# tahaspc82442/federated_multi_modal

Measured on AMD Instinct MI355X. Metric: images/sec/node (ViT-B/16 MaPLe fwd+bwd), higher is better.
Workload: dtype fp16; 1 GPU; c4: PatternNet-shape 38-class synthetic, J=9, batch=32 per client (configs[3]); clients=1, batch_per_client=32, global_batch=32, classes=38, prompt_depth=9, n_ctx=2, parallelism=one federated client per GPU x1, FedAvg all-reduce per round, round=512 local steps + 1 FedAvg, hipgraph=True

## Files before the change

federated_multi_modal_amd/_lib.py:

```python
from __future__ import annotations

import ctypes
import os
from pathlib import Path

_HERE = Path(__file__).resolve().parent
LIB_PATH = _HERE / "lib" / "libmapfed.so"

P, I, L, F = ctypes.c_void_p, ctypes.c_int, ctypes.c_int64, ctypes.c_float

SIGNATURES = {
    "mf_abi_version": [],
    "mf_gemm_nt": [P, L, P, L, P, L, I, I, I, P, P, P, L, I, I, P],
    "mf_gemm": [P, L, I, P, L, I, P, L, I, I, I, P, P, P, L, I, I, P],
    "mf_layernorm_fwd": [P, L, P, P, P, P, L, P, P, I, I, P],
    "mf_layernorm_bwd_blocks": [I],
    "mf_layernorm_bwd": [P, L, P, L, P, P, P, P, P, L, P, L, P, P, P, I, I, I, P],
    "mf_col_reduce_desc_bytes": [],
    "mf_col_reduce_batch": [P, I, I, P],
    "mf_attention_fwd": [P, L, P, L, P, I, I, I, I, I, P],
    "mf_attention_fwd_rows": [P, L, P, L, P, I, I, I, I, I, I, P],
    "mf_attention_bwd": [P, L, P, L, P, L, P, P, I, P, L, I, I, I, I, P],
    "mf_qkv_attention_fwd": [P, L, I, P, P, P, L, P, L, P, I, I, I, I, I, P],
    "mf_qkv_attention_supported": [I, I, I, I],
    "mf_im2col_patch": [P, I, P, I, I, I, P],
    "mf_vision_assemble": [P, P, P, P, P, I, I, I, I, P],
    "mf_text_assemble": [P, P, P, P, P, I, I, I, I, P],
    "mf_prompt_inject_fwd": [P, P, I, I, I, I, I, P],
    "mf_prompt_inject_bwd": [P, I, I, I, I, I, P, I, I, I, P],
    "mf_transpose_f16": [P, L, P, L, I, I, P],
    "mf_colsum_blocks": [I],
    "mf_colsum_f16": [P, L, I, I, P, I, P, P],
    "mf_cast_f16_f32": [P, P, L, P],
    "mf_small_linear_fwd": [P, P, P, P, I, I, I, I, P],
    "mf_small_linear_bwd": [P, P, P, P, P, P, I, I, I, I, I, P],
    "mf_gemm_splitk_ws_floats": [I, I, I, I],
    "mf_small_linear_desc_bytes": [],
# ... 37 lines not shown
_LIB = None


class MapfedError(RuntimeError):
    pass


def lib():
    global _LIB
    if _LIB is not None:
        return _LIB
    path = os.environ.get("MAPFED_LIB", str(LIB_PATH))
    if not os.path.exists(path):
        raise MapfedError(f"libmapfed.so not found at {path}: run __graft_entry__.build() "
                          "(make -C federated_multi_modal_amd/csrc)")
    h = ctypes.CDLL(path)
    h.mf_last_error.restype = ctypes.c_char_p
    h.mf_last_error.argtypes = []
    for name, args in SIGNATURES.items():
        fn = getattr(h, name)
        fn.argtypes = args
        fn.restype = _RESTYPES.get(name, ctypes.c_int)
    _LIB = h
    return h


def exported_symbols():
    return ["mf_last_error"] + list(SIGNATURES)


# ... 9 lines not shown
```

federated_multi_modal_amd/csrc/attention.hip:

```cpp
#include <algorithm>
#include <cstdlib>

#include "mf_common.h"

namespace {

MF_DEV int sw_off(int row, int col) {
  return row * 64 + ((((col >> 3) ^ (row & 7))) << 3) + (col & 7);
}

MF_DEV f16x4 tr_read(const f16* img, int r0, int c0, int lane) {
  const int ii = lane & 15;
  const int row = r0 + (ii >> 2);
  const int col = c0 + 4 * (ii & 3);
  const f16* p = img + sw_off(row, col);
  s16x4 v = __builtin_amdgcn_ds_read_tr16_b64_v4i16((__attribute__((address_space(3))) s16x4*)(p));
  return __builtin_bit_cast(f16x4, v);
}

MF_DEV f16x8 cat8(f16x4 a, f16x4 b) {
  return (f16x8){a[0], a[1], a[2], a[3], b[0], b[1], b[2], b[3]};
}

MF_DEV f16x8 ld_frag(const f16* img, int row, int chunk) {
  return *(const f16x8*)(img + row * 64 + ((chunk ^ (row & 7)) << 3));
}

typedef __attribute__((address_space(3))) void* lds_ptr_t;
template <int LP>
MF_DEV void stage_rows(f16* img, const f16* base, int64_t ld, int L, int col0) {
  const int lane = threadIdx.x & 63, w = threadIdx.x >> 6, nw = blockDim.x >> 6;
  const int lrow = lane >> 3, lchunk = (lane & 7) ^ lrow;
  for (int i = w; i < LP / 8; i += nw) {
    int row = i * 8 + lrow;
    row = row < L ? row : L - 1;
    __builtin_amdgcn_global_load_lds((const void*)(base + (int64_t)row * ld + col0 + lchunk * 8),
                                     (lds_ptr_t)(img + i * 8 * 64), 16, 0, 0);
  }
}
MF_DEV void stage_wait() {
  __builtin_amdgcn_s_waitcnt((0 & 15) | (7 << 4) | (15 << 8));
  __syncthreads();
}

constexpr float kScale = 0.125f;

#ifdef MF_ATTN_STAMPS
__device__ unsigned long long* g_astamps;
#define MF_ASTAMP(slot)                                                                   \
  do {                                                                                    \
    if (threadIdx.x == 0 && blockIdx.y == 0) g_astamps[(size_t)blockIdx.x * 8 + (slot)] = __builtin_amdgcn_s_memrealtime(); \
  } while (0)
// ... 609 lines not shown
}

template <int LP>
struct BwdLds {
  static constexpr int P = LP + 8;
  static constexpr int ELEMS = 2 * LP * 64 + LP * P + 2 * LP * 2;
};

MF_DEV f16x4 tr_read_p(const f16* img, int pitch, int r0, int c0, int lane) {
  const int ii = lane & 15;
  const f16* p = img + (r0 + (ii >> 2)) * pitch + c0 + 4 * (ii & 3);
  s16x4 v = __builtin_amdgcn_ds_read_tr16_b64_v4i16((__attribute__((address_space(3))) s16x4*)(p));
  return __builtin_bit_cast(f16x4, v);
}

template <int LP, bool CAUSAL, int KT>
__global__ __launch_bounds__(64 * (LP / (16 * KT))) void attn_bwd_fused_kernel(
    const f16* __restrict__ qkv, int64_t ld_qkv, const f16* __restrict__ out, int64_t ld_out,
    const f16* __restrict__ dout, int64_t ld_dout, const float* __restrict__ lse, int ld_lse,
    f16* __restrict__ dqkv, int64_t ld_dqkv, int L, int H) {
  constexpr int PT = BwdLds<LP>::P;
  __shared__ __attribute__((aligned(16))) f16 smem[BwdLds<LP>::ELEMS];
  f16* sQ = smem;
  f16* sdO = smem + LP * 64;
  f16* sdST = smem + 2 * LP * 64;
  float* sL = (float*)(sdST + LP * PT);
  float* sD = sL + LP;

  const int D = H * 64;
  const int nh = blockIdx.x, n = nh / H, h = nh % H;
  const f16* base = qkv + (int64_t)n * L * ld_qkv;
  const f16* obase = out + (int64_t)n * L * ld_out;
  const f16* dobase = dout + (int64_t)n * L * ld_dout;
  MF_ASTAMP(0);
  stage_rows<LP>(sQ, base, ld_qkv, L, h * 64);
  stage_rows<LP>(sdO, dobase, ld_dout, L, h * 64);

  const int lane = threadIdx.x & 63, w = threadIdx.x >> 6;
  const int fr = lane & 15, fg = lane >> 4;
  {
    constexpr int LPQ = 4 / KT, DPL = 64 / LPQ;
    const int q = 16 * KT * w + lane / LPQ;
    const int part = lane % LPQ;
    float d = 0.f;
    if (q < L) {
      const f16* o = obase + (int64_t)q * ld_out + h * 64 + DPL * part;
      const f16* g = dobase + (int64_t)q * ld_dout + h * 64 + DPL * part;
#pragma unroll
      for (int c = 0; c < DPL / 8; ++c) {
        f16x8 a = *(const f16x8*)(o + 8 * c), b = *(const f16x8*)(g + 8 * c);
#pragma unroll
        for (int e = 0; e < 8; ++e) d += (float)a[e] * (float)b[e];
      }
    }
#pragma unroll
    for (int o2 = 1; o2 < LPQ; o2 <<= 1) d += __shfl_xor(d, o2, 64);
    if (part == 0) {
      sD[q] = q < L ? d : 0.f;
      sL[q] = q < L ? lse[(int64_t)nh * ld_lse + q] * 1.4426950408889634f : INFINITY;
    }
  }
  const int k0 = 16 * KT * w;
  f16x8 kf[KT][2], vf[KT][2];
#pragma unroll
  for (int kt = 0; kt < KT; ++kt) {
    const int key = k0 + 16 * kt + fr;
    const int kc = key < L ? key : L - 1;
#pragma unroll
    for (int s2 = 0; s2 < 2; ++s2) {
      kf[kt][s2] = *(const f16x8*)(base + (int64_t)kc * ld_qkv + D + h * 64 + 32 * s2 + 8 * fg);
      vf[kt][s2] = *(const f16x8*)(base + (int64_t)kc * ld_qkv + 2 * D + h * 64 + 32 * s2 + 8 * fg);
    }
  }
  stage_wait();
  MF_ASTAMP(1);

  f32x4 dv[KT][4], dk[KT][4];
#pragma unroll
  for (int kt = 0; kt < KT; ++kt)
#pragma unroll
    for (int dt = 0; dt < 4; ++dt) dv[kt][dt] = dk[kt][dt] = (f32x4){0.f, 0.f, 0.f, 0.f};
#pragma unroll 1
  for (int qp = 0; qp < LP / 32; ++qp) {
    if (CAUSAL && 32 * qp + 31 < k0) continue;
    f16x8 pf[KT], dsf[KT];
#pragma unroll
    for (int a = 0; a < 2; ++a) {
      const int qt = 2 * qp + a;
      f32x4 sacc[KT], pacc[KT];
#pragma unroll
      for (int kt = 0; kt < KT; ++kt) sacc[kt] = pacc[kt] = (f32x4){0.f, 0.f, 0.f, 0.f};
#pragma unroll
      for (int s2 = 0; s2 < 2; ++s2) {
        const f16x8 qfr = ld_frag(sQ, qt * 16 + fr, 4 * s2 + fg);
        const f16x8 ofr = ld_frag(sdO, qt * 16 + fr, 4 * s2 + fg);
#pragma unroll
        for (int kt = 0; kt < KT; ++kt) {
          sacc[kt] = __builtin_amdgcn_mfma_f32_16x16x32_f16(qfr, kf[kt][s2], sacc[kt], 0, 0, 0);
// ... 57 lines not shown
    const int row = k0 + 16 * kt + fr;
#pragma unroll
    for (int s2 = 0; s2 < 2; ++s2) *(f16x8*)(sQ + row * 64 + (((4 * s2 + fg) ^ (row & 7)) << 3)) = kf[kt][s2];
  }
  __syncthreads();
  MF_ASTAMP(3);
  const f16* sK = sQ;
  const int q0 = 16 * KT * w;
  f32x4 dq[KT][4];
#pragma unroll
  for (int qt = 0; qt < KT; ++qt)
#pragma unroll
    for (int dt = 0; dt < 4; ++dt) dq[qt][dt] = (f32x4){0.f, 0.f, 0.f, 0.f};
#pragma unroll 1
  for (int ks = 0; ks < LP / 32; ++ks) {
    if (CAUSAL && 32 * ks > q0 + 16 * KT - 1) break;
    f16x8 dsf[KT];
#pragma unroll
    for (int qt = 0; qt < KT; ++qt)
      dsf[qt] = cat8(tr_read_p(sdST, PT, 32 * ks + 4 * fg, q0 + 16 * qt, lane),
                     tr_read_p(sdST, PT, 32 * ks + 16 + 4 * fg, q0 + 16 * qt, lane));
#pragma unroll
    for (int dt = 0; dt < 4; ++dt) {
      const f16x8 ak = cat8(tr_read(sK, 32 * ks + 4 * fg, 16 * dt, lane), tr_read(sK, 32 * ks + 16 + 4 * fg, 16 * dt, lane));
#pragma unroll
      for (int qt = 0; qt < KT; ++qt) dq[qt][dt] = __builtin_amdgcn_mfma_f32_16x16x32_f16(ak, dsf[qt], dq[qt][dt], 0, 0, 0);
    }
  }
#pragma unroll
  for (int qt = 0; qt < KT; ++qt) {
// ... 188 lines not shown
  attn_bwd_dkv_kernel<P, false><<<grid, block, 0, st>>>((const f16*)qkv, ld_qkv, (const f16*)dout, ld_dout, lse,     \
                                                      dq_dot_ws, ld_lse, (f16*)dqkv, ld_dqkv, L, H);               \
  attn_bwd_dq_kernel<P, false><<<grid, block, 0, st>>>((const f16*)qkv, ld_qkv, (const f16*)dout, ld_dout, lse,      \
                                                     dq_dot_ws, ld_lse, (f16*)dqkv, ld_dqkv, L, H);
    MF_ATTN_DISPATCH_LONG(LP, CALLBL)
#undef CALLBL
    MF_CHECK_LAUNCH();
    return 0;
  }
  if (LP <= 224) {
    const dim3 gridf(N * H), blockf(64 * (LP / 16));
#define CALLBF(P)                                                                                                  \
  if (causal)                                                                                                      \
    attn_bwd_fused_kernel<P, true, 1><<<gridf, blockf, 0, st>>>((const f16*)qkv, ld_qkv, (const f16*)out, ld_out,  \
                                                              (const f16*)dout, ld_dout, lse, ld_lse, (f16*)dqkv,   \
                                                              ld_dqkv, L, H);                                      \
  else                                                                                                             \
    attn_bwd_fused_kernel<P, false, 1><<<gridf, blockf, 0, st>>>((const f16*)qkv, ld_qkv, (const f16*)out, ld_out, \
                                                               (const f16*)dout, ld_dout, lse, ld_lse, (f16*)dqkv,  \
                                                               ld_dqkv, L, H);
    switch (LP) {
      case 32: CALLBF(32); break;
      case 64: CALLBF(64); break;
      case 96: CALLBF(96); break;
      case 128: CALLBF(128); break;
      case 160: CALLBF(160); break;
      case 192: CALLBF(192); break;
      case 224: CALLBF(224); break;
      default: return mf_set_error("attention: bad padded length", -1);
    }
#undef CALLBF
    MF_CHECK_LAUNCH();
    return 0;
  }
  const int64_t tot = (int64_t)N * H * L;
// ... 3 lines not shown
  const dim3 grid(N * H, attn_qsplit(N * H, L)), block(attn_threads(L));
#define CALLB(P)                                                                                                 \
  if (causal) {                                                                                                  \
    attn_bwd_dkv_kernel<P, true><<<grid, block, 0, st>>>((const f16*)qkv, ld_qkv, (const f16*)dout, ld_dout, lse,    \
                                                       dq_dot_ws, ld_lse, (f16*)dqkv, ld_dqkv, L, H);              \
    attn_bwd_dq_kernel<P, true><<<grid, block, 0, st>>>((const f16*)qkv, ld_qkv, (const f16*)dout, ld_dout, lse,     \
                                                      dq_dot_ws, ld_lse, (f16*)dqkv, ld_dqkv, L, H);               \
  } else {                                                                                                       \
    attn_bwd_dkv_kernel<P, false><<<grid, block, 0, st>>>((const f16*)qkv, ld_qkv, (const f16*)dout, ld_dout, lse,   \
                                                        dq_dot_ws, ld_lse, (f16*)dqkv, ld_dqkv, L, H);             \
    attn_bwd_dq_kernel<P, false><<<grid, block, 0, st>>>((const f16*)qkv, ld_qkv, (const f16*)dout, ld_dout, lse,    \
                                                       dq_dot_ws, ld_lse, (f16*)dqkv, ld_dqkv, L, H);              \
  }
  MF_ATTN_DISPATCH(LP, CALLB)
#undef CALLB
  MF_CHECK_LAUNCH();
  return 0;
}

extern "C" int mf_qkv_attention_fwd(const void* x, int64_t ld_x, int x_rows, const void* w, const void* bias,
                                    void* qkv, int64_t ld_qkv, void* out, int64_t ld_out, float* lse, int ld_lse,
                                    int N, int L, int H, int causal, void* stream) {
  if (N <= 0) return 0;
  const int D = H * 64;
  if ((ld_x % 8) || (ld_qkv % 8) || (ld_out % 4) || ld_lse < L || ld_x < D || ld_qkv < 3 * D ||
      (uintptr_t)x % 16 || (uintptr_t)w % 16 || (uintptr_t)qkv % 16 || (uintptr_t)bias % 8)
    return mf_set_error("mf_qkv_attention_fwd: bad strides / alignment", -1);
  if (x_rows < N * L) return mf_set_error("mf_qkv_attention_fwd: x has fewer than N*L rows", -1);
  hipStream_t st = (hipStream_t)stream;
  if (D == 768 && !causal && L > 192 && L <= 208) {
// ... 20 lines not shown
```

federated_multi_modal_amd/csrc/gemm.hip:

```cpp
#include <algorithm>
#include <cstdlib>
#include <type_traits>

#include "mf_common.h"

namespace {

enum Epi : int {
  EPI_NONE = 0,
  EPI_BIAS = 1,
  EPI_BIAS_RESID = 2,
  EPI_BIAS_GELU = 3,
  EPI_DGELU = 4,
  EPI_F32 = 5,
  EPI_RESID = 6,
};

struct GemmArgs {
  const f16* A;
  const f16* B;
  void* C;
  const f16* bias;
  const f16* aux_in;
  f16* aux_out;
// ... 1050 lines not shown
}

int launch_tile8f(const GemmArgs& a, int epi, hipStream_t st) {
  const int tiles = ((a.M + 255) / 256) * ((a.N + 255) / 256);
  dim3 grid(tiles), block(512);
  switch (epi) {
    case EPI_NONE: gemm8f_kernel<EPI_NONE><<<grid, block, 0, st>>>(a); break;
    case EPI_BIAS: gemm8f_kernel<EPI_BIAS><<<grid, block, 0, st>>>(a); break;
    case EPI_BIAS_RESID: gemm8f_kernel<EPI_BIAS_RESID><<<grid, block, 0, st>>>(a); break;
    case EPI_BIAS_GELU: gemm8f_kernel<EPI_BIAS_GELU><<<grid, block, 0, st>>>(a); break;
    case EPI_DGELU: gemm8f_kernel<EPI_DGELU><<<grid, block, 0, st>>>(a); break;
    case EPI_F32: gemm8f_kernel<EPI_F32><<<grid, block, 0, st>>>(a); break;
    case EPI_RESID: gemm8f_kernel<EPI_RESID><<<grid, block, 0, st>>>(a); break;
    default: return mf_set_error("mf_gemm_nt: bad epilogue", -2);
  }
  MF_CHECK_LAUNCH();
  return 0;
}

template <int BM, int BN, int WM, int WN>
int launch_tile8(const GemmArgs& a, int epi, hipStream_t st) {
  const int tiles = ((a.M + BM - 1) / BM) * ((a.N + BN - 1) / BN);
  dim3 grid(tiles), block(512);
  switch (epi) {
    case EPI_NONE: gemm8_kernel<BM, BN, WM, WN, EPI_NONE><<<grid, block, 0, st>>>(a); break;
    case EPI_BIAS: gemm8_kernel<BM, BN, WM, WN, EPI_BIAS><<<grid, block, 0, st>>>(a); break;
    case EPI_BIAS_RESID: gemm8_kernel<BM, BN, WM, WN, EPI_BIAS_RESID><<<grid, block, 0, st>>>(a); break;
    case EPI_BIAS_GELU: gemm8_kernel<BM, BN, WM, WN, EPI_BIAS_GELU><<<grid, block, 0, st>>>(a); break;
    case EPI_DGELU: gemm8_kernel<BM, BN, WM, WN, EPI_DGELU><<<grid, block, 0, st>>>(a); break;
    case EPI_F32: gemm8_kernel<BM, BN, WM, WN, EPI_F32><<<grid, block, 0, st>>>(a); break;
// ... 93 lines not shown
    return mf_set_error("mf_gemm: epilogue needs aux_in", -1);
  const int vec8 = (ldc % 8 == 0) && (ld_aux % 8 == 0) && ((uintptr_t)C % 16 == 0) &&
                   (!aux_in || (uintptr_t)aux_in % 16 == 0) && (!aux_out || (uintptr_t)aux_out % 16 == 0);
  GemmArgs a{(const f16*)A, (const f16*)B, C, (const f16*)bias, (const f16*)aux_in, (f16*)aux_out,
             lda, ldb, ldc, ld_aux, M, N, K, vec8, 0, gemm_xcd_split(M, N, K)};
  hipStream_t st = (hipStream_t)stream;
  const int64_t t128 = (int64_t)((M + 127) / 128) * ((N + 127) / 128);
  if (a_kmajor || b_kmajor) {
    if (tile <= 0) tile = t128 >= 512 ? 1 : (t128 >= 256 ? 2 : 3);
    return launch_kmajor(a, a_kmajor != 0, b_kmajor != 0, epilogue, tile, st);
  }
  const bool side = tile == -1 && M >= 2048;
  if (tile == -1) tile = side ? kSideTile : 0;
  if (tile == 0) {
    const int64_t t256 = (int64_t)((M + 255) / 256) * ((N + 255) / 256);
    if (t256 >= 192 && t256 <= 256 && K >= 512)
      tile = 40;
    else if (M >= 16384 && K >= 512)
      tile = (N >= 1536 || K >= 1024 || (N >= 768 && K >= 768)) ? 40 : 10;
    else if (M >= 4096 && K >= 512)
      tile = N > 1024 ? 10 : (K >= 2048 ? 15 : 16);
    else if (M >= 2048 && N >= 1024 && K <= 768)
      tile = N >= 2048 ? 15 : 26;
    else if (M >= 2048 && N <= 768 && K >= 512)
      tile = 26;
    else if (M < 2048 && K >= 512) {
      const int64_t t64 = (int64_t)((M + 63) / 64) * ((N + 63) / 64);
      if (K >= 1536) tile = t64 >= 128 ? 31 : 33;
      else if (N >= 3072 || (N > 1024 && N < 2048)) tile = 26;
      else tile = 3;
    } else
// ... 3 lines not shown
    case 1: return launch_tile<128, 128, 2, 2, 2>(a, epilogue, st);
    case 2: return launch_tile<128, 64, 2, 2, 2>(a, epilogue, st);
    case 3: return launch_tile<64, 64, 2, 2, 2>(a, epilogue, st);
    case 10: return launch_tile<160, 128, 2, 2, 2>(a, epilogue, st);
    case 11: return launch_tile<160, 128, 2, 2, 3>(a, epilogue, st);
    case 15: return launch_tile<96, 128, 2, 2, 2>(a, epilogue, st);
    case 16: return launch_tile<160, 64, 2, 2, 2>(a, epilogue, st);
    case 26: return launch_tile<96, 64, 2, 2, 2>(a, epilogue, st);
    case 31: return launch_tile<64, 64, 2, 2, 4>(a, epilogue, st);
    case 33: return launch_tile<32, 64, 2, 2, 4>(a, epilogue, st);
    case 20: return K < 128 ? launch_tile<128, 128, 2, 2, 2>(a, epilogue, st) : launch_tile8s(a, epilogue, st);
    case 21: return K < 128 ? launch_tile<128, 128, 2, 2, 2>(a, epilogue, st) : launch_tile8<256, 128, 2, 4>(a, epilogue, st);
    case 22: return K < 128 ? launch_tile<128, 128, 2, 2, 2>(a, epilogue, st) : launch_tile8<256, 256, 2, 4>(a, epilogue, st);
    case 40: return K < 128 ? launch_tile<128, 128, 2, 2, 2>(a, epilogue, st) : launch_tile8f(a, epilogue, st);
    case 41: return K < 128 ? launch_tile<128, 128, 2, 2, 2>(a, epilogue, st) : launch_tile8p(a, epilogue, st);
    default: return mf_set_error("mf_gemm: bad tile id", -2);
  }
}

extern "C" int mf_gemm_nt(const void* A, int64_t lda, const void* B, int64_t ldb, void* C, int64_t ldc, int M,
                          int N, int K, const void* bias, const void* aux_in, void* aux_out, int64_t ld_aux,
                          int epilogue, int tile, void* stream) {
  return mf_gemm(A, lda, 0, B, ldb, 0, C, ldc, M, N, K, bias, aux_in, aux_out, ld_aux, epilogue, tile, stream);
}

extern "C" int mf_gemm_splitk(const void* A, int64_t lda, int a_kmajor, const void* B, int64_t ldb, int b_kmajor,
                              void* C, int64_t ldc, int M, int N, int K, float* ws, int64_t ws_floats, int splits,
                              int out_f16, void* stream) {
  if (M <= 0 || N <= 0) return 0;
  const bool both_k = a_kmajor && b_kmajor;
// ... 40 lines not shown
```

federated_multi_modal_amd/engine.py:

```python
from __future__ import annotations

import math
import os
from dataclasses import dataclass, field
from typing import Dict, List, Optional, Tuple

import numpy as np
import torch

from . import ops
from . import synthetic as syn
from .tokenizer import get_tokenizer

F16, F32 = torch.float16, torch.float32
N_CTX = 2


@dataclass
class EngineConfig:
    batch: int
    classnames: List[str]
    prompt_depth: int = 9
    seed: int = 0
    n_ctx: int = N_CTX
# ... 164 lines not shown
        self.layers, self.causal, self.row0 = layers, causal, inject_row0
        self.Ls = list(Ls) if Ls is not None else [L] * layers
        assert len(self.Ls) == layers and self.Ls[0] == L
        self.ncap = ncap
        self.grow = [i > 0 and self.Ls[i] != self.Ls[i - 1] for i in range(layers)]
        assert not any(self.grow) or all(self.Ls[i] - self.Ls[i - 1] in (0, ncap) for i in range(1, layers))
        self.L_out = self.Ls[-1]
        dev = eng.device
        Rs = [N * l for l in self.Ls]
        self.Rs = Rs
        R = max(Rs)
        self.R = R
        e = lambda *s, dt=F16: torch.empty(*s, device=dev, dtype=dt)
        self.inference = bool(eng.cfg.inference)
        self.cls_only = False
        if self.inference:
            if any(self.grow):
                raise NotImplementedError("EngineConfig.inference with growing (caption) sequences")
            self._alloc_forward_only(e, R, N, H, D, layers)
            return
        self.X = [e(Rs[0], D)]
        self.Y = []
        for i in range(layers):
            if i + 1 < layers and self.grow[i + 1]:
                self.Y.append(e(Rs[i], D))
                self.X.append(e(Rs[i + 1], D))
            else:
                self.X.append(e(Rs[i], D))
                self.Y.append(self.X[i + 1])
        self.QKV = [e(Rs[i], 3 * D) for i in range(layers)]
# ... 48 lines not shown
        self.tile = 0
        self.lnb = self.cs_ws = self.dw_ws = None
        self.dw_split = set()

    def p(self, i: int, key: str) -> torch.Tensor:
        return self.e.P[f"{self.name}.transformer.resblocks.{i}.{key}"]

    def wt(self, i: int, key: str) -> torch.Tensor:
        return self.e.WT[f"{self.name}.transformer.resblocks.{i}.{key}"]

    def g(self, i: int, key: str) -> torch.Tensor:
        return self.e.G[f"{self.name}.transformer.resblocks.{i}.{key}"]

    def forward(self, deep_prompts: List[torch.Tensor], cap: Optional[torch.Tensor] = None):
        N, D, H = self.N, self.D, self.H
        for i in range(self.layers):
            L, R = self.Ls[i], self.Rs[i]
            x = self.X[i]
            h1 = self.H1[:R]
            if 1 <= i <= len(deep_prompts) and not self.grow[i]:
                ops.layernorm_fwd_inject(x, self.p(i, "ln_1.weight"), self.p(i, "ln_1.bias"), h1, self.mean1[i],
                                         self.rstd1[i], deep_prompts[i - 1], L, self.row0, N_CTX)
            else:
                ops.layernorm_fwd(x, self.p(i, "ln_1.weight"), self.p(i, "ln_1.bias"), h1, self.mean1[i],
                                  self.rstd1[i])
            if self.cls_only and i == self.layers - 1:
                self._last_block_cls_rows(i, x, h1, L)
                continue
            if self.fused_qkv_attn and ops.qkv_attention_supported(N, L, H, self.causal):
                ops.qkv_attention_fwd(h1, self.p(i, "attn.in_proj_weight"), self.p(i, "attn.in_proj_bias"),
                                      self.QKV[i], self.O[i], self.LSE[i], N, L, H, self.causal)
            else:
                ops.gemm_nt(h1, self.p(i, "attn.in_proj_weight"), self.QKV[i], bias=self.p(i, "attn.in_proj_bias"),
                            epilogue=ops.EPI_BIAS, tile=self.tile)
                ops.attention_fwd(self.QKV[i], N, L, H, self.causal, out=self.O[i], lse=self.LSE[i])
            h2 = self.H2[:R]
            ops.gemm_nt(self.O[i], self.p(i, "attn.out_proj.weight"), self.X1[i],
                        bias=self.p(i, "attn.out_proj.bias"), aux_in=x, epilogue=ops.EPI_BIAS_RESID, tile=self.tile)
            ops.layernorm_fwd(self.X1[i], self.p(i, "ln_2.weight"), self.p(i, "ln_2.bias"), h2, self.mean2[i],
                              self.rstd2[i])
            g = self.G[:R]
            ops.gemm_nt(h2, self.p(i, "mlp.c_fc.weight"), g, bias=self.p(i, "mlp.c_fc.bias"),
# ... 9 lines not shown
        ops.gemm_nt(h1, w[D:], self.QKV[i][:, D:], bias=b[D:], epilogue=ops.EPI_BIAS, tile=self.tile)
        ops.gemm_nt(h1[::L], w[:D], self.QKV[i][::L, :D], bias=b[:D], epilogue=ops.EPI_BIAS, tile=self.tile)
        ops.attention_fwd_rows(self.QKV[i], N, L, H, self.causal, 1, out=self.O[i], lse=self.LSE[i])
        x1 = self.X1[i][::L]
        ops.gemm_nt(self.O[i][::L], self.p(i, "attn.out_proj.weight"), x1, bias=self.p(i, "attn.out_proj.bias"),
                    aux_in=x[::L], epilogue=ops.EPI_BIAS_RESID, tile=self.tile)
        h2 = self.H2[:N]
        ops.layernorm_fwd(x1, self.p(i, "ln_2.weight"), self.p(i, "ln_2.bias"), h2, self.mean2[i][:N],
                          self.rstd2[i][:N])
        g = self.G[:N]
        ops.gemm_nt(h2, self.p(i, "mlp.c_fc.weight"), g, bias=self.p(i, "mlp.c_fc.bias"), epilogue=ops.EPI_BIAS_GELU,
                    tile=self.tile)
        ops.gemm_nt(g, self.p(i, "mlp.c_proj.weight"), self.Y[i][::L], bias=self.p(i, "mlp.c_proj.bias"), aux_in=x1,
                    epilogue=ops.EPI_BIAS_RESID, tile=self.tile)

    def _dw(self, dY: torch.Tensor, Xin: torch.Tensor, dW: torch.Tensor, db: torch.Tensor):
        if self.live is not None:
            Ll, Lf = self.live
            for src, full in ((dY, self.full_dy), (Xin, self.full_x)):
                assert src.shape[0] == self.N * Ll and src.shape[1] <= full.shape[1] and full.shape[0] == self.N * Lf
            dY = ops.seq_scatter(dY, self.full_dy[:, :dY.shape[1]], self.N, Ll, Lf)[:self.N * Lf]
            Xin = ops.seq_scatter(Xin, self.full_x[:, :Xin.shape[1]], self.N, Ll, Lf)[:self.N * Lf]
        if tuple(dW.shape) in self.dw_split:
            ops.gemm_splitk(dY, Xin, dW, self.dw_ws, a_kmajor=True, b_kmajor=True)
        else:
            ops.gemm(dY, Xin, dW, epilogue=ops.EPI_NONE, a_kmajor=True, b_kmajor=True)
        ops.colsum(dY, db, self.cs_ws)

    def backward(self, n_prompted: int, prompt_grads: List[torch.Tensor]):
        if self.inference:
            raise RuntimeError("backward on a forward-only (EngineConfig.inference) engine")
        N, D, H = self.N, self.D, self.H
        last = self.layers - 1
        for i in reversed(range(self.layers)):
            L, R = self.Ls[i], self.Rs[i]
            dX = self.dX[:R]
            dF, dH, dO, dQKV = self.dF[:R], self.dH[:R], self.dO[:R], self.dQKV[:R]
            trainable_w = i == last
            ops.gemm_nt(dX, self.wt(i, "mlp.c_proj.weight"), dF, aux_in=self.Fp[i], epilogue=ops.EPI_DGELU,
                        tile=self.tile)
            if trainable_w:
                self._dw(dX, self.G[:R], self.g(i, "mlp.c_proj.weight"), self.g(i, "mlp.c_proj.bias"))
            ops.gemm_nt(dF, self.wt(i, "mlp.c_fc.weight"), dH, epilogue=ops.EPI_NONE, tile=self.tile)
            if trainable_w:
                self._dw(dF, self.H2[:R], self.g(i, "mlp.c_fc.weight"), self.g(i, "mlp.c_fc.bias"))
            self.lnb.bwd(dH, self.X1[i], self.p(i, "ln_2.weight"), self.mean2[i], self.rstd2[i], dX,
                         self.g(i, "ln_2.weight"), self.g(i, "ln_2.bias"), dres=dX, live=self.live)
            ops.gemm_nt(dX, self.wt(i, "attn.out_proj.weight"), dO, epilogue=ops.EPI_NONE, tile=self.tile)
            if trainable_w:
                self._dw(dX, self.O[i], self.g(i, "attn.out_proj.weight"), self.g(i, "attn.out_proj.bias"))
            ops.attention_bwd(self.QKV[i], self.O[i], dO, self.LSE[i], N, L, H, self.causal, dqkv=dQKV,
                              ws=self.attn_ws)
            ops.gemm_nt(dQKV, self.wt(i, "attn.in_proj_weight"), dH, epilogue=ops.EPI_NONE, tile=self.tile)
            if trainable_w:
                self._dw(dQKV, self.H1[:R], self.g(i, "attn.in_proj_weight"), self.g(i, "attn.in_proj_bias"))
            if 1 <= i <= n_prompted and not self.grow[i]:
                self.lnb.bwd_inject(dH, self.X[i], self.p(i, "ln_1.weight"), self.mean1[i], self.rstd1[i], dX,
                                    self.g(i, "ln_1.weight"), self.g(i, "ln_1.bias"), dX, prompt_grads[i - 1], L,
                                    self.row0, N_CTX, live=self.live)
            else:
                self.lnb.bwd(dH, self.X[i], self.p(i, "ln_1.weight"), self.mean1[i], self.rstd1[i], dX,
                             self.g(i, "ln_1.weight"), self.g(i, "ln_1.bias"), dres=dX, live=self.live)
            if self.grow[i]:
                ops.prompt_inject_bwd(dX, N, L, L - N_CTX, N_CTX, D, prompt_grads[i - 1], accumulate=False,
                                      zero_rows=False)
                Lp = self.Ls[i - 1]
                ops.seq_grow_bwd(dX, self.dX2[:N * Lp], N, Lp, self.ncap, N_CTX, D)
# ... 43 lines not shown
            if max(Ls) > 512:
                raise NotImplementedError(f"caption path: vision sequence of {max(Ls)} rows (> 512) at B={self.B}, "
                                          f"J={self.J}")
        self.vis = _Tower(self, "image_encoder", self.B, self.Lv, d.vision_width, d.vision_heads, d.vision_layers,
                          False, G2 + 1, Ls=Ls, ncap=self.B if cfg.captions else 0)
        self.txt = _Tower(self, "text_encoder", self.K, self.text_len, d.text_width, d.text_heads, d.text_layers,
                          True, 1, L_full=d.context_length)
        self._build_io()
        vis_work = self.vis.N * self.vis.L * self.vis.D ** 2
        txt_work = self.txt.N * self.txt.L * self.txt.D ** 2
        (self.txt if txt_work <= vis_work else self.vis).tile = -1
        if cfg.fused_qkv_attn == "side":
            for t in (self.vis, self.txt):
                t.fused_qkv_attn = t.tile == -1 and t.Rs[0] >= 2048
        self.vis.cls_only = bool(cfg.inference) and not cfg.captions
        self.side = torch.cuda.Stream(device=self.device)
        self.overlap_towers = True
        self.vision_first = cfg.vision_first
        self.step_count = 0
        self.momentum_initialised = False

    def _build_params(self, vals: Dict[str, np.ndarray]):
        dev = self.device
        tr16 = [(n, s) for n, s, dt in self.specs if _is_trainable(n) and dt == F16 and "proj_vis_to_lang" not in n]
        tr32 = [(n, s) for n, s, dt in self.specs if _is_trainable(n) and dt == F32]
        n16 = sum(int(np.prod(s)) for _, s in tr16)
        n32 = sum(int(np.prod(s)) for _, s in tr32)
        self.n16, self.n32 = n16, n32
        self.flat16 = torch.empty(n16, device=dev, dtype=F16)
        self.flat32 = torch.empty(n32, device=dev, dtype=F32)
# ... 301 lines not shown
                  self.dXpre, G["image_encoder.ln_pre.weight"], G["image_encoder.ln_pre.bias"])
        ops.prompt_inject_bwd(self.dXpre, self.B, self.Lv, self.G2 + 1, N_CTX, v.D, self.g_shared_ctx,
                              accumulate=False, zero_rows=False)
        v.lnb.finish()

    def forward_loss(self):
        self.input_flag.zero_()
        ops.nonfinite_flag(self.img_in, self.input_flag)
        if self.soft_labels:
            ops.nonfinite_flag(self.soft_label_in, self.input_flag)
        main = torch.cuda.current_stream(self.device)
        side = self.side if self.overlap_towers else main
        side.wait_stream(main)
        with torch.cuda.stream(side):
            self.refresh_transposes(all_layers=False)
        self.forward()
        if self.soft_labels:
            ops.clip_loss_soft_fwd_bwd(self.img_feat, self.txt_feat, self.img_n, self.txt_n, self.norms,
                                       self.logits, self.soft_label_in, self.P["logit_scale"], self.dmm, self.cos_ws,
                                       self.soft_ws, self.loss_out, self.dimg_n, self.dtxt_n, self.dimg, self.dtxt)
        else:
            ops.clip_loss_fwd_bwd(self.img_feat, self.txt_feat, self.img_n, self.txt_n, self.norms, self.logits,
                                  self.label_in, self.P["logit_scale"], self.dmm, self.cos_ws, self.loss_out,
                                  self.dimg_n, self.dtxt_n, self.dimg, self.dtxt)

    def backward(self):
        main = torch.cuda.current_stream(self.device)
        side = self.side if self.overlap_towers else main
        side.wait_stream(main)
        if self.vision_first:
            self._vision_backward()
# ... 141 lines not shown
```

federated_multi_modal_amd/ops.py:

```python
from __future__ import annotations

import ctypes
import os
from typing import Optional

import torch

from ._lib import call

EPI_NONE, EPI_BIAS, EPI_BIAS_RESID, EPI_BIAS_GELU, EPI_DGELU, EPI_F32, EPI_RESID = range(7)


class KernelProbe:

    def __init__(self, kinds="gemm"):
        self.kinds = {kinds} if isinstance(kinds, str) else set(kinds)
        self.kind = next(iter(self.kinds)) if len(self.kinds) == 1 else None
        self.records = []

    def wants(self, kind: str) -> bool:
        return kind in self.kinds

    def around(self, flops: float, nbytes: float, key: str = "gemm", meta=None):
        s = torch.cuda.Event(enable_timing=True)
# ... 355 lines not shown


def attention_bwd(qkv, out, dout, lse, N, L, H, causal, dqkv=None, ws=None, ld_lse=None):
    if ld_lse is None:
        ld_lse = L
    if dqkv is None:
        dqkv = torch.empty_like(qkv)
    if ws is None:
        ws = torch.empty(N * H * ld_lse, device=qkv.device, dtype=torch.float32)
    ev = None
    if _PROBE is not None and _PROBE.wants("attention"):
        pairs = L * (L + 1) / 2 if causal else L * L
        ev = _PROBE.around(8.0 * N * H * pairs * 64, N * H * L * (2.0 * 8 * 64 + 4), f"attention_bwd/L{L}")
    call("mf_attention_bwd", _p(qkv), _ld(qkv), _p(out), _ld(out), _p(dout), _ld(dout), _p(lse), _p(ws), ld_lse,
         _p(dqkv), _ld(dqkv), N, L, H, int(causal), _s())
    if ev is not None:
        ev.record()
    return dqkv


def im2col_patch(img, out, patch=16):
    B, C, R, R2 = img.shape
    assert C == 3 and R == R2 and img.is_contiguous()
    call("mf_im2col_patch", _p(img), int(img.dtype == torch.float32), _p(out), B, R, patch, _s())
    return out


def vision_assemble(patch, cls, pos, shared_ctx, x, B, G2, n_ctx, D):
    call("mf_vision_assemble", _p(patch), _p(cls), _p(pos), _p(shared_ctx), _p(x), B, G2, n_ctx, D, _s())
    return x
# ... 321 lines not shown
```

include/mapfed.h:

```cpp
#ifndef MAPFED_H_
#define MAPFED_H_
#include <stdint.h>

#ifdef __cplusplus
extern "C" {
#endif

const char* mf_last_error(void);
int mf_abi_version(void);

int mf_gemm_nt(const void* A, int64_t lda, const void* B, int64_t ldb, void* C, int64_t ldc, int M, int N, int K,
               const void* bias, const void* aux_in, void* aux_out, int64_t ld_aux, int epilogue, int tile,
               void* stream);
int mf_gemm(const void* A, int64_t lda, int a_kmajor, const void* B, int64_t ldb, int b_kmajor, void* C, int64_t ldc,
            int M, int N, int K, const void* bias, const void* aux_in, void* aux_out, int64_t ld_aux, int epilogue,
            int tile, void* stream);
int mf_gemm_splitk(const void* A, int64_t lda, int a_kmajor, const void* B, int64_t ldb, int b_kmajor, void* C,
                   int64_t ldc, int M, int N, int K, float* ws, int64_t ws_floats, int splits, int out_f16,
                   void* stream);
int mf_gemm_splitk_ws_floats(int M, int N, int K, int splits);

int mf_layernorm_fwd(const void* x, int64_t ldx, const int* row_index, const float* gamma, const float* beta,
                     void* y, int64_t ldy, float* mean, float* rstd, int rows, int D, void* stream);
int mf_layernorm_fwd_inject(void* x, int64_t ldx, const float* gamma, const float* beta, void* y, int64_t ldy,
// ... 17 lines not shown

int mf_col_reduce_desc_bytes(void);
int mf_col_reduce_batch(const void* descs, int n, int max_cols, void* stream);

int mf_attention_fwd(const void* qkv, int64_t ld_qkv, void* out, int64_t ld_out, float* lse, int ld_lse, int N,
                     int L, int H, int causal, void* stream);
int mf_attention_fwd_rows(const void* qkv, int64_t ld_qkv, void* out, int64_t ld_out, float* lse, int ld_lse, int N,
                          int L, int H, int causal, int q_rows, void* stream);
int mf_qkv_attention_fwd(const void* x, int64_t ld_x, int x_rows, const void* w, const void* bias, void* qkv,
                         int64_t ld_qkv, void* out, int64_t ld_out, float* lse, int ld_lse, int N, int L, int H,
                         int causal, void* stream);
int mf_qkv_attention_supported(int N, int L, int H, int causal);
int mf_attention_bwd(const void* qkv, int64_t ld_qkv, const void* out, int64_t ld_out, const void* dout,
                     int64_t ld_dout, const float* lse, float* dq_dot_ws, int ld_lse, void* dqkv, int64_t ld_dqkv,
                     int N, int L, int H, int causal, void* stream);

int mf_im2col_patch(const void* img, int img_is_f32, void* out, int B, int R, int P, void* stream);
int mf_vision_assemble(const void* patch, const float* cls, const float* pos, const void* shared_ctx, void* x,
                       int B, int G2, int n_ctx, int D, void* stream);
int mf_text_assemble(const void* prefix, const void* ctx, const void* suffix, const float* pos, void* x, int K,
                     int L, int n_ctx, int D, void* stream);
int mf_prompt_inject_fwd(void* x, const float* prompt, int N, int L, int row0, int nrows, int D, void* stream);
int mf_prompt_inject_bwd(void* dx, int N, int L, int row0, int nrows, int D, void* out, int out_f16, int accumulate,
                         int zero_rows, void* stream);

int mf_seq_grow(const void* src, void* dst, const void* cap, const float* prompt, int N, int Lp, int ncap, int n_ctx,
                int D, void* stream);
int mf_seq_grow_bwd(const void* ddst, void* dsrc, int N, int Lp, int ncap, int n_ctx, int D, void* stream);
int mf_caption_pool(const int* tokens, int B, int T, const float* table, int vocab, const void* w, int D,
                    void* pooled, void* stream);
// ... 72 lines not shown
```

Before: 5596 images/s.

## Compute only CLS rows in last vision block during training, add small-M GEMM

```diff
diff --git a/federated_multi_modal_amd/_lib.py b/federated_multi_modal_amd/_lib.py
--- a/federated_multi_modal_amd/_lib.py
+++ b/federated_multi_modal_amd/_lib.py
@@ -21,6 +21,7 @@
     "mf_attention_fwd": [P, L, P, L, P, I, I, I, I, I, P],
     "mf_attention_fwd_rows": [P, L, P, L, P, I, I, I, I, I, I, P],
     "mf_attention_bwd": [P, L, P, L, P, L, P, P, I, P, L, I, I, I, I, P],
+    "mf_attention_bwd_rows": [P, L, P, L, P, L, P, I, P, L, I, I, I, I, I, P],
     "mf_qkv_attention_fwd": [P, L, I, P, P, P, L, P, L, P, I, I, I, I, I, P],
     "mf_qkv_attention_supported": [I, I, I, I],
     "mf_im2col_patch": [P, I, P, I, I, I, P],
@@ -88,6 +89,7 @@
     if not os.path.exists(path):
         raise MapfedError(f"libmapfed.so not found at {path}: run __graft_entry__.build() "
                           "(make -C federated_multi_modal_amd/csrc)")
+    import torch
     h = ctypes.CDLL(path)
     h.mf_last_error.restype = ctypes.c_char_p
     h.mf_last_error.argtypes = []
diff --git a/federated_multi_modal_amd/csrc/attention.hip b/federated_multi_modal_amd/csrc/attention.hip
--- a/federated_multi_modal_amd/csrc/attention.hip
+++ b/federated_multi_modal_amd/csrc/attention.hip
@@ -36,6 +36,26 @@
     row = row < L ? row : L - 1;
     __builtin_amdgcn_global_load_lds((const void*)(base + (int64_t)row * ld + col0 + lchunk * 8),
                                      (lds_ptr_t)(img + i * 8 * 64), 16, 0, 0);
+  }
+}
+MF_DEV void stage_rows_n(f16* img, const f16* base, int64_t ld, int L, int col0, int ng) {
+  const int lane = threadIdx.x & 63, w = threadIdx.x >> 6, nw = blockDim.x >> 6;
+  const int lrow = lane >> 3, lchunk = (lane & 7) ^ lrow;
+  for (int i = w; i < ng; i += nw) {
+    int row = i * 8 + lrow;
+    row = row < L ? row : L - 1;
+    __builtin_amdgcn_global_load_lds((const void*)(base + (int64_t)row * ld + col0 + lchunk * 8),
+                                     (lds_ptr_t)(img + i * 8 * 64), 16, 0, 0);
+  }
+}
+MF_DEV void stage_rows_live(f16* img, const f16* base, int64_t ld, int live, int col0, int ng) {
+  const int lane = threadIdx.x & 63, w = threadIdx.x >> 6, nw = blockDim.x >> 6;
+  const int lrow = lane >> 3, lchunk = (lane & 7) ^ lrow;
+  for (int i = w; i < ng; i += nw) {
+    const int row = i * 8 + lrow;
+    f16x8 v = {0, 0, 0, 0, 0, 0, 0, 0};
+    if (row < live) v = *(const f16x8*)(base + (int64_t)row * ld + col0 + lchunk * 8);
+    *(f16x8*)(img + i * 8 * 64 + lane * 8) = v;
   }
 }
 MF_DEV void stage_wait() {
@@ -675,12 +695,14 @@
   return __builtin_bit_cast(f16x4, v);
 }
 
-template <int LP, bool CAUSAL, int KT>
+template <int LP, bool CAUSAL, int KT, bool ROWS = false>
 __global__ __launch_bounds__(64 * (LP / (16 * KT))) void attn_bwd_fused_kernel(
     const f16* __restrict__ qkv, int64_t ld_qkv, const f16* __restrict__ out, int64_t ld_out,
     const f16* __restrict__ dout, int64_t ld_dout, const float* __restrict__ lse, int ld_lse,
-    f16* __restrict__ dqkv, int64_t ld_dqkv, int L, int H) {
+    f16* __restrict__ dqkv, int64_t ld_dqkv, int L, int H, int q_rows) {
   constexpr int PT = BwdLds<LP>::P;
+  const int live = ROWS ? q_rows : L;
+  const int nqb = ROWS ? (q_rows + 31) / 32 : LP / 32;
   __shared__ __attribute__((aligned(16))) f16 smem[BwdLds<LP>::ELEMS];
   f16* sQ = smem;
   f16* sdO = smem + LP * 64;
@@ -694,8 +716,13 @@
   const f16* obase = out + (int64_t)n * L * ld_out;
   const f16* dobase = dout + (int64_t)n * L * ld_dout;
   MF_ASTAMP(0);
-  stage_rows<LP>(sQ, base, ld_qkv, L, h * 64);
-  stage_rows<LP>(sdO, dobase, ld_dout, L, h * 64);
+  if (ROWS) {
+    stage_rows_n(sQ, base, ld_qkv, L, h * 64, 4 * nqb);
+    stage_rows_live(sdO, dobase, ld_dout, live, h * 64, 4 * nqb);
+  } else {
+    stage_rows<LP>(sQ, base, ld_qkv, L, h * 64);
+    stage_rows<LP>(sdO, dobase, ld_dout, L, h * 64);
+  }
 
   const int lane = threadIdx.x & 63, w = threadIdx.x >> 6;
   const int fr = lane & 15, fg = lane >> 4;
@@ -704,7 +731,7 @@
     const int q = 16 * KT * w + lane / LPQ;
     const int part = lane % LPQ;
     float d = 0.f;
-    if (q < L) {
+    if (q < live) {
       const f16* o = obase + (int64_t)q * ld_out + h * 64 + DPL * part;
       const f16* g = dobase + (int64_t)q * ld_dout + h * 64 + DPL * part;
 #pragma unroll
@@ -717,8 +744,8 @@
 #pragma unroll
     for (int o2 = 1; o2 < LPQ; o2 <<= 1) d += __shfl_xor(d, o2, 64);
     if (part == 0) {
-      sD[q] = q < L ? d : 0.f;
-      sL[q] = q < L ? lse[(int64_t)nh * ld_lse + q] * 1.4426950408889634f : INFINITY;
+      sD[q] = q < live ? d : 0.f;
+      sL[q] = q < live ? lse[(int64_t)nh * ld_lse + q] * 1.4426950408889634f : INFINITY;
     }
   }
   const int k0 = 16 * KT * w;
@@ -742,7 +769,7 @@
 #pragma unroll
     for (int dt = 0; dt < 4; ++dt) dv[kt][dt] = dk[kt][dt] = (f32x4){0.f, 0.f, 0.f, 0.f};
 #pragma unroll 1
-  for (int qp = 0; qp < LP / 32; ++qp) {
+  for (int qp = 0; qp < nqb; ++qp) {
     if (CAUSAL && 32 * qp + 31 < k0) continue;
     f16x8 pf[KT], dsf[KT];
 #pragma unroll
@@ -830,6 +857,7 @@
     for (int dt = 0; dt < 4; ++dt) dq[qt][dt] = (f32x4){0.f, 0.f, 0.f, 0.f};
 #pragma unroll 1
   for (int ks = 0; ks < LP / 32; ++ks) {
+    if (ROWS && q0 >= q_rows) break;
     if (CAUSAL && 32 * ks > q0 + 16 * KT - 1) break;
     f16x8 dsf[KT];
 #pragma unroll
@@ -1048,11 +1076,11 @@
   if (causal)                                                                                                      \
     attn_bwd_fused_kernel<P, true, 1><<<gridf, blockf, 0, st>>>((const f16*)qkv, ld_qkv, (const f16*)out, ld_out,  \
                                                               (const f16*)dout, ld_dout, lse, ld_lse, (f16*)dqkv,   \
-                                                              ld_dqkv, L, H);                                      \
+                                                              ld_dqkv, L, H, L);                                   \
   else                                                                                                             \
     attn_bwd_fused_kernel<P, false, 1><<<gridf, blockf, 0, st>>>((const f16*)qkv, ld_qkv, (const f16*)out, ld_out, \
                                                                (const f16*)dout, ld_dout, lse, ld_lse, (f16*)dqkv,  \
-                                                               ld_dqkv, L, H);
+                                                               ld_dqkv, L, H, L);
     switch (LP) {
       case 32: CALLBF(32); break;
       case 64: CALLBF(64); break;
@@ -1086,6 +1114,37 @@
   }
   MF_ATTN_DISPATCH(LP, CALLB)
 #undef CALLB
+  MF_CHECK_LAUNCH();
+  return 0;
+}
+
+extern "C" int mf_attention_bwd_rows(const void* qkv, int64_t ld_qkv, const void* out, int64_t ld_out,
+                                     const void* dout, int64_t ld_dout, const float* lse, int ld_lse, void* dqkv,
+                                     int64_t ld_dqkv, int N, int L, int H, int causal, int q_rows, void* stream) {
+  if (N <= 0) return 0;
+  if (L <= 0 || L > 224) return mf_set_error("mf_attention_bwd_rows: 0 < L <= 224 required", -1);
+  if (causal) return mf_set_error("mf_attention_bwd_rows: causal masks are not supported", -1);
+  if (q_rows <= 0 || q_rows > L) return mf_set_error("mf_attention_bwd_rows: 0 < q_rows <= L required", -1);
+  if (ld_lse < L || (ld_qkv % 8) || (ld_out % 8) || (ld_dout % 8) || (ld_dqkv % 4))
+    return mf_set_error("mf_attention_bwd_rows: bad strides", -1);
+  const int LP = padded_len(L);
+  hipStream_t st = (hipStream_t)stream;
+  const dim3 gridf(N * H), blockf(64 * (LP / 16));
+#define CALLBR(P)                                                                                                     \
+  attn_bwd_fused_kernel<P, false, 1, true><<<gridf, blockf, 0, st>>>((const f16*)qkv, ld_qkv, (const f16*)out, ld_out, \
+                                                                     (const f16*)dout, ld_dout, lse, ld_lse,         \
+                                                                     (f16*)dqkv, ld_dqkv, L, H, q_rows);
+  switch (LP) {
+    case 32: CALLBR(32); break;
+    case 64: CALLBR(64); break;
+    case 96: CALLBR(96); break;
+    case 128: CALLBR(128); break;
+    case 160: CALLBR(160); break;
+    case 192: CALLBR(192); break;
+    case 224: CALLBR(224); break;
+    default: return mf_set_error("attention: bad padded length", -1);
+  }
+#undef CALLBR
   MF_CHECK_LAUNCH();
   return 0;
 }
diff --git a/federated_multi_modal_amd/csrc/gemm.hip b/federated_multi_modal_amd/csrc/gemm.hip
--- a/federated_multi_modal_amd/csrc/gemm.hip
+++ b/federated_multi_modal_amd/csrc/gemm.hip
@@ -1088,6 +1088,81 @@
     case EPI_RESID: gemm8f_kernel<EPI_RESID><<<grid, block, 0, st>>>(a); break;
     default: return mf_set_error("mf_gemm_nt: bad epilogue", -2);
   }
+  MF_CHECK_LAUNCH();
+  return 0;
+}
+
+constexpr int SM_NW = 8;
+template <int PS, int EPI>
+__global__ __launch_bounds__(SM_NW * 64) void gemm_sm_kernel(GemmArgs g) {
+  __shared__ __attribute__((aligned(16))) float s_acc[2][64][4];
+  __shared__ __attribute__((aligned(16))) f16 s_c[32 * (16 + 8)];
+  const int tid = threadIdx.x, lane = tid & 63;
+  const int wid = __builtin_amdgcn_readfirstlane(tid >> 6);
+  const int fr = lane & 15, fg = lane >> 4;
+  const int n0 = blockIdx.x * 16, m0 = blockIdx.y * 32;
+  const int steps = g.K / 32;
+  const int s0 = wid * PS;
+  const int ns = min(PS, steps - s0);
+  const bool two = m0 + 16 < g.M;
+  const f16* wrow = g.B + (int64_t)min(n0 + fr, g.N - 1) * g.ldb + 8 * fg;
+  const f16* arow0 = g.A + (int64_t)min(m0 + fr, g.M - 1) * g.lda + 8 * fg;
+  const f16* arow1 = g.A + (int64_t)min(m0 + 16 + fr, g.M - 1) * g.lda + 8 * fg;
+  f16x8 wf[PS], af0[PS], af1[PS];
+#pragma unroll
+  for (int s = 0; s < PS; ++s) {
+    wf[s] = af0[s] = af1[s] = f16x8{};
+    if (s < ns) {
+      const int k = (s0 + s) * 32;
+      wf[s] = *(const f16x8*)(wrow + k);
+      af0[s] = *(const f16x8*)(arow0 + k);
+      if (two) af1[s] = *(const f16x8*)(arow1 + k);
+    }
+  }
+  const int turns = (steps + PS - 1) / PS;
+  for (int t = 0; t < turns; ++t) {
+    if (wid == t) {
+      f32x4 a0 = {0.f, 0.f, 0.f, 0.f}, a1 = {0.f, 0.f, 0.f, 0.f};
+      if (t > 0) {
+        a0 = *(const f32x4*)s_acc[0][lane];
+        a1 = *(const f32x4*)s_acc[1][lane];
+      }
+#pragma unroll
+      for (int s = 0; s < PS; ++s) {
+        if (s < ns) {
+          a0 = __builtin_amdgcn_mfma_f32_16x16x32_f16(wf[s], af0[s], a0, 0, 0, 0);
+          if (two) a1 = __builtin_amdgcn_mfma_f32_16x16x32_f16(wf[s], af1[s], a1, 0, 0, 0);
+        }
+      }
+      *(f32x4*)s_acc[0][lane] = a0;
+      *(f32x4*)s_acc[1][lane] = a1;
+    }
+    __syncthreads();
+  }
+  f32x4 fin[1][1];
+  fin[0][0] = *(const f32x4*)s_acc[wid & 1][lane];
+  epilogue_store<32, 16, SM_NW * 64, 1, 1, EPI>(g, s_c, fin, m0, n0, 16 * (wid & 1), 0, tid, fr, fg);
+}
+
+int launch_small_m(const GemmArgs& a, int epi, hipStream_t st) {
+  if (a.M > 64 || a.K > 12 * 32 * SM_NW) return mf_set_error("mf_gemm: tile 50 needs M <= 64 and K <= 3072", -2);
+  dim3 grid((a.N + 15) / 16, (a.M + 31) / 32), block(SM_NW * 64);
+#define MF_SM(E)                                                       \
+  case E:                                                              \
+    if (a.K <= 4 * 32 * SM_NW) gemm_sm_kernel<4, E><<<grid, block, 0, st>>>(a); \
+    else gemm_sm_kernel<12, E><<<grid, block, 0, st>>>(a);             \
+    break;
+  switch (epi) {
+    MF_SM(EPI_NONE)
+    MF_SM(EPI_BIAS)
+    MF_SM(EPI_BIAS_RESID)
+    MF_SM(EPI_BIAS_GELU)
+    MF_SM(EPI_DGELU)
+    MF_SM(EPI_F32)
+    MF_SM(EPI_RESID)
+    default: return mf_set_error("mf_gemm: bad epilogue", -2);
+  }
+#undef MF_SM
   MF_CHECK_LAUNCH();
   return 0;
 }
@@ -1211,7 +1286,9 @@
   if (tile == -1) tile = side ? kSideTile : 0;
   if (tile == 0) {
     const int64_t t256 = (int64_t)((M + 255) / 256) * ((N + 255) / 256);
-    if (t256 >= 192 && t256 <= 256 && K >= 512)
+    if (M <= 64 && K <= 3072)
+      tile = 50;
+    else if (t256 >= 192 && t256 <= 256 && K >= 512)
       tile = 40;
     else if (M >= 16384 && K >= 512)
       tile = (N >= 1536 || K >= 1024 || (N >= 768 && K >= 768)) ? 40 : 10;
@@ -1245,6 +1322,7 @@
     case 22: return K < 128 ? launch_tile<128, 128, 2, 2, 2>(a, epilogue, st) : launch_tile8<256, 256, 2, 4>(a, epilogue, st);
     case 40: return K < 128 ? launch_tile<128, 128, 2, 2, 2>(a, epilogue, st) : launch_tile8f(a, epilogue, st);
     case 41: return K < 128 ? launch_tile<128, 128, 2, 2, 2>(a, epilogue, st) : launch_tile8p(a, epilogue, st);
+    case 50: return launch_small_m(a, epilogue, st);
     default: return mf_set_error("mf_gemm: bad tile id", -2);
   }
 }
diff --git a/federated_multi_modal_amd/engine.py b/federated_multi_modal_amd/engine.py
--- a/federated_multi_modal_amd/engine.py
+++ b/federated_multi_modal_amd/engine.py
@@ -202,6 +202,10 @@
         e = lambda *s, dt=F16: torch.empty(*s, device=dev, dtype=dt)
         self.inference = bool(eng.cfg.inference)
         self.cls_only = False
+        self.train_cls_rows = False
+        self._cls_pass = False
+        self._cls_fwd = False
+        self.cls_G = self.cls_H2 = self.cls_dF = None
         if self.inference:
             if any(self.grow):
                 raise NotImplementedError("EngineConfig.inference with growing (caption) sequences")
@@ -280,6 +284,7 @@
 
     def forward(self, deep_prompts: List[torch.Tensor], cap: Optional[torch.Tensor] = None):
         N, D, H = self.N, self.D, self.H
+        self._cls_fwd = self.train_cls_rows and self._cls_pass
         for i in range(self.layers):
             L, R = self.Ls[i], self.Rs[i]
             x = self.X[i]
@@ -292,6 +297,9 @@
                                   self.rstd1[i])
             if self.cls_only and i == self.layers - 1:
                 self._last_block_cls_rows(i, x, h1, L)
+                continue
+            if self._cls_fwd and i == self.layers - 1:
+                self._last_block_train_cls_rows(i, x, h1, L)
                 continue
             if self.fused_qkv_attn and ops.qkv_attention_supported(N, L, H, self.causal):
                 ops.qkv_attention_fwd(h1, self.p(i, "attn.in_proj_weight"), self.p(i, "attn.in_proj_bias"),
@@ -331,6 +339,46 @@
         ops.gemm_nt(g, self.p(i, "mlp.c_proj.weight"), self.Y[i][::L], bias=self.p(i, "mlp.c_proj.bias"), aux_in=x1,
                     epilogue=ops.EPI_BIAS_RESID, tile=self.tile)
 
+    def enable_train_cls_rows(self):
+        assert not self.inference and not any(self.grow) and self.live is None and not self.causal and self.L <= 224
+        z = lambda c: torch.zeros(self.R, c, device=self.e.device, dtype=F16)
+        self.cls_G, self.cls_H2, self.cls_dF = z(4 * self.D), z(self.D), z(4 * self.D)
+        self.O[-1].zero_()
+        self.train_cls_rows = True
+
+    def _last_block_train_cls_rows(self, i: int, x: torch.Tensor, h1: torch.Tensor, L: int):
+        N, H = self.N, self.H
+        ops.gemm_nt(h1, self.p(i, "attn.in_proj_weight"), self.QKV[i], bias=self.p(i, "attn.in_proj_bias"),
+                    epilogue=ops.EPI_BIAS, tile=self.tile)
+        ops.attention_fwd_rows(self.QKV[i], N, L, H, self.causal, 1, out=self.O[i], lse=self.LSE[i])
+        x1 = self.X1[i][::L]
+        ops.gemm_nt(self.O[i][::L], self.p(i, "attn.out_proj.weight"), x1, bias=self.p(i, "attn.out_proj.bias"),
+                    aux_in=x[::L], epilogue=ops.EPI_BIAS_RESID, tile=self.tile)
+        h2 = self.cls_H2[::L]
+        ops.layernorm_fwd(x1, self.p(i, "ln_2.weight"), self.p(i, "ln_2.bias"), h2, self.mean2[i][:N],
+                          self.rstd2[i][:N])
+        g = self.cls_G[::L]
+        ops.gemm_nt(h2, self.p(i, "mlp.c_fc.weight"), g, bias=self.p(i, "mlp.c_fc.bias"), aux_out=self.Fp[i][::L],
+                    epilogue=ops.EPI_BIAS_GELU, tile=self.tile)
+        ops.gemm_nt(g, self.p(i, "mlp.c_proj.weight"), self.Y[i][::L], bias=self.p(i, "mlp.c_proj.bias"), aux_in=x1,
+                    epilogue=ops.EPI_BIAS_RESID, tile=self.tile)
+
+    def _last_block_bwd_cls_rows(self, i: int, L: int, R: int):
+        N, H = self.N, self.H
+        dX = self.dX[:R]
+        dXc, dFc, dHc = dX[::L], self.cls_dF[:R][::L], self.dH[:R][::L]
+        ops.gemm_nt(dXc, self.wt(i, "mlp.c_proj.weight"), dFc, aux_in=self.Fp[i][::L], epilogue=ops.EPI_DGELU,
+                    tile=self.tile)
+        self._dw(dX, self.cls_G[:R], self.g(i, "mlp.c_proj.weight"), self.g(i, "mlp.c_proj.bias"))
+        ops.gemm_nt(dFc, self.wt(i, "mlp.c_fc.weight"), dHc, epilogue=ops.EPI_NONE, tile=self.tile)
+        self._dw(self.cls_dF[:R], self.cls_H2[:R], self.g(i, "mlp.c_fc.weight"), self.g(i, "mlp.c_fc.bias"))
+        self.lnb.bwd(dHc, self.X1[i][::L], self.p(i, "ln_2.weight"), self.mean2[i][:N], self.rstd2[i][:N], dXc,
+                     self.g(i, "ln_2.weight"), self.g(i, "ln_2.bias"), dres=dXc, live=(1, L))
+        ops.gemm_nt(dXc, self.wt(i, "attn.out_proj.weight"), self.dO[:R][::L], epilogue=ops.EPI_NONE, tile=self.tile)
+        self._dw(dX, self.O[i], self.g(i, "attn.out_proj.weight"), self.g(i, "attn.out_proj.bias"))
+        ops.attention_bwd_rows(self.QKV[i], self.O[i], self.dO[:R], self.LSE[i], N, L, H, self.causal, 1,
+                               dqkv=self.dQKV[:R])
+
     def _dw(self, dY: torch.Tensor, Xin: torch.Tensor, dW: torch.Tensor, db: torch.Tensor):
         if self.live is not None:
             Ll, Lf = self.live
@@ -354,20 +402,23 @@
             dX = self.dX[:R]
             dF, dH, dO, dQKV = self.dF[:R], self.dH[:R], self.dO[:R], self.dQKV[:R]
             trainable_w = i == last
-            ops.gemm_nt(dX, self.wt(i, "mlp.c_proj.weight"), dF, aux_in=self.Fp[i], epilogue=ops.EPI_DGELU,
-                        tile=self.tile)
-            if trainable_w:
-                self._dw(dX, self.G[:R], self.g(i, "mlp.c_proj.weight"), self.g(i, "mlp.c_proj.bias"))
-            ops.gemm_nt(dF, self.wt(i, "mlp.c_fc.weight"), dH, epilogue=ops.EPI_NONE, tile=self.tile)
-            if trainable_w:
-                self._dw(dF, self.H2[:R], self.g(i, "mlp.c_fc.weight"), self.g(i, "mlp.c_fc.bias"))
-            self.lnb.bwd(dH, self.X1[i], self.p(i, "ln_2.weight"), self.mean2[i], self.rstd2[i], dX,
-                         self.g(i, "ln_2.weight"), self.g(i, "ln_2.bias"), dres=dX, live=self.live)
-            ops.gemm_nt(dX, self.wt(i, "attn.out_proj.weight"), dO, epilogue=ops.EPI_NONE, tile=self.tile)
-            if trainable_w:
-                self._dw(dX, self.O[i], self.g(i, "attn.out_proj.weight"), self.g(i, "attn.out_proj.bias"))
-            ops.attention_bwd(self.QKV[i], self.O[i], dO, self.LSE[i], N, L, H, self.causal, dqkv=dQKV,
-                              ws=self.attn_ws)
+            if trainable_w and self._cls_fwd:
+                self._last_block_bwd_cls_rows(i, L, R)
+            else:
+                ops.gemm_nt(dX, self.wt(i, "mlp.c_proj.weight"), dF, aux_in=self.Fp[i], epilogue=ops.EPI_DGELU,
+                            tile=self.tile)
+                if trainable_w:
+                    self._dw(dX, self.G[:R], self.g(i, "mlp.c_proj.weight"), self.g(i, "mlp.c_proj.bias"))
+                ops.gemm_nt(dF, self.wt(i, "mlp.c_fc.weight"), dH, epilogue=ops.EPI_NONE, tile=self.tile)
+                if trainable_w:
+                    self._dw(dF, self.H2[:R], self.g(i, "mlp.c_fc.weight"), self.g(i, "mlp.c_fc.bias"))
+                self.lnb.bwd(dH, self.X1[i], self.p(i, "ln_2.weight"), self.mean2[i], self.rstd2[i], dX,
+                             self.g(i, "ln_2.weight"), self.g(i, "ln_2.bias"), dres=dX, live=self.live)
+                ops.gemm_nt(dX, self.wt(i, "attn.out_proj.weight"), dO, epilogue=ops.EPI_NONE, tile=self.tile)
+                if trainable_w:
+                    self._dw(dX, self.O[i], self.g(i, "attn.out_proj.weight"), self.g(i, "attn.out_proj.bias"))
+                ops.attention_bwd(self.QKV[i], self.O[i], dO, self.LSE[i], N, L, H, self.causal, dqkv=dQKV,
+                                  ws=self.attn_ws)
             ops.gemm_nt(dQKV, self.wt(i, "attn.in_proj_weight"), dH, epilogue=ops.EPI_NONE, tile=self.tile)
             if trainable_w:
                 self._dw(dQKV, self.H1[:R], self.g(i, "attn.in_proj_weight"), self.g(i, "attn.in_proj_bias"))
@@ -441,6 +492,8 @@
             for t in (self.vis, self.txt):
                 t.fused_qkv_attn = t.tile == -1 and t.Rs[0] >= 2048
         self.vis.cls_only = bool(cfg.inference) and not cfg.captions
+        if not cfg.inference and not cfg.captions and self.Lv <= 224:
+            self.vis.enable_train_cls_rows()
         self.side = torch.cuda.Stream(device=self.device)
         self.overlap_towers = True
         self.vision_first = cfg.vision_first
@@ -772,7 +825,11 @@
         side.wait_stream(main)
         with torch.cuda.stream(side):
             self.refresh_transposes(all_layers=False)
-        self.forward()
+        self.vis._cls_pass = True
+        try:
+            self.forward()
+        finally:
+            self.vis._cls_pass = False
         if self.soft_labels:
             ops.clip_loss_soft_fwd_bwd(self.img_feat, self.txt_feat, self.img_n, self.txt_n, self.norms,
                                        self.logits, self.soft_label_in, self.P["logit_scale"], self.dmm, self.cos_ws,
diff --git a/federated_multi_modal_amd/ops.py b/federated_multi_modal_amd/ops.py
--- a/federated_multi_modal_amd/ops.py
+++ b/federated_multi_modal_amd/ops.py
@@ -393,6 +393,23 @@
         ev = _PROBE.around(8.0 * N * H * pairs * 64, N * H * L * (2.0 * 8 * 64 + 4), f"attention_bwd/L{L}")
     call("mf_attention_bwd", _p(qkv), _ld(qkv), _p(out), _ld(out), _p(dout), _ld(dout), _p(lse), _p(ws), ld_lse,
          _p(dqkv), _ld(dqkv), N, L, H, int(causal), _s())
+    if ev is not None:
+        ev.record()
+    return dqkv
+
+
+def attention_bwd_rows(qkv, out, dout, lse, N, L, H, causal, q_rows, dqkv=None, ld_lse=None):
+    if ld_lse is None:
+        ld_lse = L
+    if dqkv is None:
+        dqkv = torch.empty_like(qkv)
+    ev = None
+    if _PROBE is not None and _PROBE.wants("attention"):
+        rows = min(L, (q_rows + 31) // 32 * 32)
+        ev = _PROBE.around(8.0 * N * H * rows * L * 64, N * H * (2.0 * 5 * 64 * L + 2.0 * 3 * 64 * rows),
+                           f"attention_bwd_rows/L{L}")
+    call("mf_attention_bwd_rows", _p(qkv), _ld(qkv), _p(out), _ld(out), _p(dout), _ld(dout), _p(lse), ld_lse,
+         _p(dqkv), _ld(dqkv), N, L, H, int(causal), q_rows, _s())
     if ev is not None:
         ev.record()
     return dqkv
diff --git a/include/mapfed.h b/include/mapfed.h
--- a/include/mapfed.h
+++ b/include/mapfed.h
@@ -55,6 +55,9 @@
 int mf_attention_bwd(const void* qkv, int64_t ld_qkv, const void* out, int64_t ld_out, const void* dout,
                      int64_t ld_dout, const float* lse, float* dq_dot_ws, int ld_lse, void* dqkv, int64_t ld_dqkv,
                      int N, int L, int H, int causal, void* stream);
+int mf_attention_bwd_rows(const void* qkv, int64_t ld_qkv, const void* out, int64_t ld_out, const void* dout,
+                          int64_t ld_dout, const float* lse, int ld_lse, void* dqkv, int64_t ld_dqkv, int N, int L,
+                          int H, int causal, int q_rows, void* stream);
 
 int mf_im2col_patch(const void* img, int img_is_f32, void* out, int B, int R, int P, void* stream);
 int mf_vision_assemble(const void* patch, const float* cls, const float* pos, const void* shared_ctx, void* x,
```

After: 5804 images/s (median of 6 runs). 3.7% higher.
